# byteowlz/kokorox

Measured on AMD Instinct MI355X. Metric: real-time factor (audio-s/wall-s), 24 kHz, batch=64, higher is better.
Workload: dtype f32 in / out, f32 accumulate; products on split operands: f16f8 (a_hi b_hi on f16 MFMAs, the cross terms a_lo b_hi + a_hi b_lo of the 7 / 11-tap convs on e4m3 scaled MFMAs: ~17 significant bits per product; every other conv f16x3: ~22) -- wider than the bf16 BASELINE configs[2] names, inside the 1e-; 1 GPU; batch=64/GPU synthetic 128-phoneme utterances (T=130), durations pinned 3,3,3,4 -> F=422 frames = 10.55 s each, noise on, inputs in HBM; batch_per_gpu=64, frames=422, parallelism=utterance-sharded x1, one-time weight broadcast

## Files before the change

### kokorox_amd/build.py

```python
from __future__ import annotations

import os
import subprocess
import sys

HERE = os.path.dirname(os.path.abspath(__file__))
CSRC = os.path.join(HERE, "csrc")
LIB_DIR = os.path.join(HERE, "lib")
LIB_PATH = os.path.join(LIB_DIR, "libkokorox_hip.so")
TEST_LIB_PATH = os.path.join(LIB_DIR, "libkokorox_hip_test.so")
TEST_SOURCES = ["test_hooks.hip"]
SOURCES = ["conv_plan.hip", "conv_mfma.hip", "conv_f16x3.hip", "conv_f16x3_da.hip", "conv_f16x3_da_p1.hip", "conv_f16x3_da_w2.hip", "conv_f16x3_da_s16.hip", "conv_f16x3_da_f8.hip", "conv_f16x3_da_pre.hip", "conv_f16x3_pre.hip", "conv_f16x3_dapn.hip", "conv_f16x3_dag.hip", "kernels_misc.hip", "model.hip", "api.hip", "dispatcher.hip", "onnx_import.cpp"]
HEADERS = ["kx_common.h", "kx_error.h", "conv_epilogue.h", "conv_f16x3_common.h"]
_PUB = os.path.join("..", "..", "include", "kokorox_hip.h")
_PUB_TEST = os.path.join("..", "..", "include", "kokorox_hip_test.h")
EXTRA_DEPS = {"model.hip": ["onnx_import.h", "model.h", _PUB], "api.hip": ["model.h", "kx_handle.h", "api_guard.h", _PUB],
              "dispatcher.hip": ["model.h", "kx_handle.h", "dispatcher_core.h", _PUB],
              "test_hooks.hip": ["model.h", "kx_handle.h", "api_guard.h", _PUB, _PUB_TEST], "onnx_import.cpp": ["onnx_import.h"], "conv_f16x3_da_p1.hip": ["conv_f16x3_da.hip"], "conv_f16x3_da_w2.hip": ["conv_f16x3_da.hip"], "conv_f16x3_da_s16.hip": ["conv_f16x3_da.hip"], "conv_f16x3_da_f8.hip": ["conv_f16x3_da.hip"], "conv_f16x3_da_pre.hip": ["conv_f16x3_da.hip"]}
FLAGS = ["-O3", "--offload-arch=gfx950", "-fPIC", "-std=c++17", "-Wall", "-Wno-unused-result"]


def _hipcc() -> str:
    for cand in (os.environ.get("HIPCC"), "/opt/rocm/bin/hipcc", "hipcc"):
        if cand and (os.path.isabs(cand) and os.path.exists(cand) or not os.path.isabs(cand)):
            return cand
    return "hipcc"


def _newer(target: str, deps) -> bool:
    if not os.path.exists(target):
        return False
    t = os.path.getmtime(target)
    return all(os.path.getmtime(d) <= t for d in deps)


LAST_BUILD = {"compiled": [], "reused": [], "linked": False}


def build_library(force: bool = False, verbose: bool = False) -> str:
    LAST_BUILD["compiled"], LAST_BUILD["reused"], LAST_BUILD["linked"] = [], [], False
    os.makedirs(LIB_DIR, exist_ok=True)
# ... 40 lines not shown
```

### kokorox_amd/csrc/conv_f16x3.hip

```cpp
#include "conv_f16x3_common.h"

namespace kx {

template <int BM, int BN, int WM, int WN, int ACT, int TK, bool PF, int VT>
__global__ __launch_bounds__(WM * WN * 64, (WM * WN == 8) ? 4 : ((BM / WM / 32) * (BN / WN / 32) > 6 ? 2 : 3))
void conv1d_f16x3_kernel(const ConvArgs a) {
    constexpr int MT = BM / WM / 32;
    constexpr int NT = BN / WN / 32;
    constexpr int NWV = WM * WN;
    static_assert((NWV == 4 || NWV == 8) && MT >= 1 && NT >= 1, "4 or 8 waves per workgroup");
    static_assert(VT == 1 || (VT <= TK && PF), "virtual taps need TK >= VT and the prefetching build");
    extern __shared__ __attribute__((aligned(16))) unsigned char smem16[];

    const int tid = threadIdx.x;
    const int lane = tid & 63;
    const int wave = __builtin_amdgcn_readfirstlane(tid >> 6);
    const int wm = wave / WN, wn = wave % WN;
    const int r = lane & 31, h = lane >> 5;
    const int b = blockIdx.z, ct = blockIdx.y;
    int tile_x = blockIdx.x;
    if (a.xcd_swizzle && gridDim.x >= 16) {
        const int nx = gridDim.x;
        const int off = (int)(((long)nx * (blockIdx.y + (long)gridDim.y * blockIdx.z)) & 7);
        const int cls = (blockIdx.x + off) & 7;
// ... 364 lines not shown
    else if (bm == 32 && bn == 256 && wm == 1 && wn == 4)
        launch_inst16<32, 256, 1, 4>(p, a, B, s);
    else
        throw Error(1, "conv1d f16x3: no such LDS-DMA form");
}

void launch_conv(const ConvPlan& p, const ConvArgs& a, int B, hipStream_t s) {
    if (p.form == FORM_F32) {
        launch_conv1d(a, p.bm, B, p.cols, s);
        return;
    }
    KX_REQUIRE(a.n_chunks16 == (a.Cin + CK16 - 1) / CK16 && a.w16 != nullptr, "conv1d f16x3: weights not packed");
    KX_REQUIRE(a.epi != EPI_GELU_NEW || p.vt > 1 || p.form == FORM_DAG || p.form == FORM_DAGN,
               "conv1d f16x3: gelu epilogue exists only for k=1 GEMMs with >= 48 input channels");
    KX_REQUIRE(p.merged == (a.merge_T > 0), "conv1d f16x3: merged columns do not match the plan");
    if (p.cols <= 0) return;
    switch (p.form) {
        case FORM_LDS: launch_lds(p, a, B, s); return;
        case FORM_DAG:
        case FORM_DAGN: launch_conv1d_f16x3_dag(p, a, B, s); return;
        case FORM_DAPN: launch_conv1d_f16x3_dapn(a, B, p.cols, s); return;
        case FORM_DA_PRE: launch_conv16_da_pre(p, a, B, s); return;
        case FORM_DA_S16: launch_conv16_da_s16(p, a, B, s); return;
        case FORM_DA_F8: launch_conv16_da_f8(p, a, B, s); return;
        case FORM_DA:
            if (p.p1) {
                launch_conv16_da_p1(p, a, B, s);
                return;
            }
            [[fallthrough]];
        case FORM_DA_W2: {
            static const int dephase = getenv("KX_DEPHASE") ? atoi(getenv("KX_DEPHASE")) : 0;
            static const int dephase_mode = getenv("KX_DEPHASE_MODE") ? atoi(getenv("KX_DEPHASE_MODE")) : 1;
            ConvArgs d;
            const ConvArgs* ap = &a;
            if (dephase > 0 && p.bn == 256) {
                d = a;
                const long grid_n = (long)((p.cols + 255) / 256) * ((a.Cout + 127) / 128) * B;
                const double tile_cycles = (double)a.n_chunks16 * a.K * 8 * 96 * 2.5 + 50000.0;
                d.dephase_cycles = grid_n >= 1024 ? (int)(tile_cycles * dephase / 1000.0) : 0;
                d.dephase_mode = dephase_mode;
                ap = &d;
            }
            if (p.form == FORM_DA_W2)
                launch_conv16_da_w2(p, *ap, B, s);
            else
                launch_conv16_da(p, *ap, B, s);
// ... 172 lines not shown
```

### kokorox_amd/csrc/conv_f16x3_da.hip

```cpp
#include "conv_f16x3_common.h"
#include <type_traits>


#ifndef KX_F8_RAW_AUX
#define KX_F8_RAW_AUX 0
#endif
#ifndef KX_F8_HWCOS
#define KX_F8_HWCOS 1
#endif

namespace kx {

template <int I, int N, class F>
__device__ __forceinline__ void static_for(F&& f) {
    if constexpr (I < N) {
        f(std::integral_constant<int, I>{});
        static_for<I + 1, N>(f);
    }
}

template <int KT, int RH, int RC, int RAW>
struct F8Sched {
    static constexpr int HS = (KT - 1) / 2, NG = (KT + 1) / 4, NC = 2 * NG;
    static constexpr int cross_of(int p) {
        if (p & 1) return -1;
        if (p <= 2 * (NG - 1)) return p / 2;
        if (p >= KT - 1 - 2 * (NG - 1)) return NC - 1 - (KT - 1 - p) / 2;
        return -1;
// ... 11 lines not shown
                n += 2;
                st_h[p + RH <= KT - 1 ? sc * KT + p + RH : (sc + 1) * KT + p % RH] = n;
                const int c = cross_of(p);
                if (c >= 0) {
                    n += 4;
                    st_x[sc * NC + c + RC] = n;
                }
            }
            n += RAW;
        }
        return result < 63 ? result : 63;
    }
    static constexpr int cum(int NB, int first, int n) {
        int t = 0;
        for (int r = 0; r < n; ++r) t += cross_of((first + r) / NB) >= 0 ? 3 : 1;
        return t;
    }
    static constexpr int hu_before(int NB, int NA, int HU, int first, int I0, int rel) {
        return rel > I0 ? ((cum(NB, first, rel) - cum(NB, first, I0)) * HU) / (cum(NB, first, NA) - cum(NB, first, I0)) : 0;
    }
};

template <int ACT, int KT, int NTT, bool P1, bool W2 = false, bool S16 = false, bool PRE = false, bool BF = false, bool F8 = false>
__global__ __launch_bounds__(256, (NTT == 8 || S16) ? 2 : 3) void conv1d_f16x3_da_kernel(const ConvArgs a) {
    static_assert(!BF || P1, "BF: a form of the reduced-precision kernels only");
    static_assert(!F8 || (S16 && KT % 4 == 3), "F8: a form of the S16 loop; tap groups of four with one padding slot");
    constexpr bool HWC = F8 && KX_F8_HWCOS;
    static_assert(!PRE || (!P1 && !S16 && ACT == ACT_NONE), "PRE: the activation lives in the image; f16x3 forms on 32x32x16 only");
    static_assert(!W2 || (KT >= 3 && (KT & 1) && NTT == 8), "W2: odd compile-time tap counts on the 256-column tile");
    static_assert(!S16 || (KT >= 3 && (KT & 1) && !P1 && !W2), "S16: odd compile-time tap counts, three MFMAs per product, 4 x 1 waves");
    static_assert(NTT == 8 || NTT == 4 || (NTT == 6 && S16), "tile widths: 256, 128, and 192 columns in the S16 form");
    constexpr int BM = 128, NT = NTT, BN = 32 * NT;
    constexpr bool W64 = KT > 0;
    constexpr bool SPLIT = W64 && BN % 128 == 0;
    constexpr int NJF = W64 ? (SPLIT ? BN / 128 : (BN + 64) / 128) : (BN + 128) / 128;
    constexpr int NJ = NJF + (SPLIT ? 1 : 0);
    constexpr int HU = 8 * NJF + (SPLIT ? 4 : 0);
    constexpr int XWp = W64 ? BN + 64 : BN + 128;
    static_assert(!W64 || SPLIT || (BN + 64) % 128 == 0, "the window is whole 64-column blocks in pairs, or ends in a split block");
    constexpr int XBUF = 4 * XWp;
    constexpr int tap_units = 4 * BM;
    extern __shared__ __attribute__((aligned(16))) unsigned char smem16[];
    uint4* Xs = reinterpret_cast<uint4*>(smem16);

    const int tid = threadIdx.x;
    const int lane = tid & 63;
    const int wave = __builtin_amdgcn_readfirstlane(tid >> 6);
    const int r = lane & 31, h = lane >> 5;
    auto pack_pair = [](float v0, float v1, unsigned& hi_pk, unsigned& lo_pk) __attribute__((always_inline)) {
        if constexpr (BF) {
            auto rne = [](float x) __attribute__((always_inline)) {
                unsigned u = __builtin_bit_cast(unsigned, x);
                u += 0x7fffu + ((u >> 16) & 1u);
                return u >> 16;
            };
            hi_pk = rne(v0) | (rne(v1) << 16);
            lo_pk = 0u;
        } else if constexpr (F8) {
            split_pair_f8(v0, v1, hi_pk, lo_pk);
        } else {
            split_pair(v0, v1, hi_pk, lo_pk);
        }
// ... 67 lines not shown
    const int K = KT > 0 ? KT : a.K, dil = a.dil;
    const int n_chunks = a.n_chunks16;
    const int n_steps = n_chunks * K;
    const float* xb = a.x + (long)b * a.x_bs;
    const int p0 = t0 - a.pad;
    const bool has_norm = a.nmean != nullptr;
    const int up2 = a.in_up2;
    const int Lsrc = up2 ? ((Lin + 1) >> 1) : Lin;

    f32x16 acc[1][NT];
#pragma unroll
    for (int j = 0; j < NT; ++j)
#pragma unroll
        for (int e = 0; e < 16; ++e) acc[0][j][e] = 0.f;
    constexpr int NB16 = S16 ? 2 * NT : 1;
    f32x4v acc16[2][NB16];
#pragma unroll
    for (int i = 0; i < 2; ++i)
#pragma unroll
        for (int j = 0; j < NB16; ++j) acc16[i][j] = f32x4v{0.f, 0.f, 0.f, 0.f};

    const int g = wave & 1, jb = wave >> 1;
    float raw[NJ][8];
    float praw[4];
    int xoff[NJ];
    unsigned okmask = 0;
    auto blk_col = [&](int j) __attribute__((always_inline)) { return (SPLIT && j == NJF) ? 64 * 2 * NJF : 64 * (jb + 2 * j); };
#pragma unroll
    for (int j = 0; j < NJ; ++j) {
        const int p = p0 + lane + blk_col(j);
        okmask |= (p >= 0 && p < Lin) ? (1u << j) : 0u;
        int pi = up2 ? (p >> 1) : p;
        pi = pi < 0 ? 0 : (pi >= Lsrc ? Lsrc - 1 : pi);
        xoff[j] = pi;
    }
    using u32x4 = __attribute__((ext_vector_type(4))) unsigned;
    constexpr int NLD = PRE ? (4 * XWp) / 256 : 1;
    static_assert(!PRE || (4 * XWp) % 256 == 0, "PRE: whole rounds of 256 lanes");
    u32x4 rawq[NLD];
    unsigned qoff[NLD];
    unsigned okq = 0;
    const buf_rsrc xq = make_buf(PRE ? reinterpret_cast<const char*>(a.x16) + (long)b * a.x16_bs : reinterpret_cast<const char*>(a.x));
    const unsigned chunk_bytes = PRE ? 64u * (unsigned)a.x16_ld : 0u;
    const buf_rsrc xrow = make_buf(xb);
    if constexpr (PRE) {
#pragma unroll
        for (int i = 0; i < NLD; ++i) {
            const int idx = tid + 256 * i, plane = idx / XWp, u = idx - plane * XWp;
            const int p = p0 + u;
            okq |= (p >= 0 && p < Lin) ? (1u << i) : 0u;
            const int pc = p < 0 ? 0 : (p >= Lin ? Lin - 1 : p);
            qoff[i] = 16u * (unsigned)(plane * a.x16_ld + pc);
        }
    }
    const int cmax_in = a.Cin - 1;
    const float* nm_src = has_norm ? a.nmean + (long)b * a.n_bs : xb;
    const float* ns_src = has_norm ? a.nscale + (long)b * a.n_bs : xb;
    const float* nh_src = has_norm ? a.nshift + (long)b * a.n_bs : xb;
    auto load_params = [&](int ch, float (&pv)[4]) __attribute__((always_inline)) {
        const int c = ch * CK16 + g * 8 + (lane & 7);
        const int cc = c < cmax_in ? c : cmax_in;
        const float m = nm_src[cc], sc = ns_src[cc], sh = nh_src[cc];
        const bool cvalid = c <= cmax_in;
        pv[0] = has_norm ? m : 0.f;
        pv[1] = cvalid ? (has_norm ? sc : 1.f) : 0.f;
        pv[2] = (cvalid && has_norm) ? sh : 0.f;
        pv[3] = (ACT == ACT_SNAKE) ? a.alpha[cc] : 1.f;
    };
    auto load_raw = [&](int ch) __attribute__((always_inline)) {
        if constexpr (PRE) {
#pragma unroll
            for (int i = 0; i < NLD; ++i)
                rawq[i] = __builtin_bit_cast(u32x4, __builtin_amdgcn_raw_buffer_load_b128(xq, qoff[i], (unsigned)ch * chunk_bytes, 0));
            return;
        }
        load_params(ch, praw);
        if constexpr (F8) {
#pragma unroll
            for (int c = 0; c < 8; ++c) {
                const int ci = ch * CK16 + g * 8 + c;
                const unsigned so = (unsigned)__builtin_amdgcn_readfirstlane(ci < cmax_in ? ci : cmax_in) * (4u * (unsigned)a.x_ld);
#pragma unroll
                for (int j = 0; j < NJF; ++j) raw[j][c] = __builtin_bit_cast(float, __builtin_amdgcn_raw_buffer_load_b32(xrow, 4u * (unsigned)xoff[j], so, KX_F8_RAW_AUX));
            }
            if constexpr (SPLIT) {
#pragma unroll
                for (int c = 0; c < 4; ++c) {
                    const int ci = ch * CK16 + g * 8 + jb * 4 + c;
                    const unsigned so = (unsigned)__builtin_amdgcn_readfirstlane(ci < cmax_in ? ci : cmax_in) * (4u * (unsigned)a.x_ld);
                    raw[NJF][c] = __builtin_bit_cast(float, __builtin_amdgcn_raw_buffer_load_b32(xrow, 4u * (unsigned)xoff[NJF], so, KX_F8_RAW_AUX));
                }
            }
            return;
        }
#pragma unroll
        for (int c = 0; c < 8; ++c) {
            const int ci = ch * CK16 + g * 8 + c;
            const float* row = xb + (long)(ci < cmax_in ? ci : cmax_in) * a.x_ld;
#pragma unroll
            for (int j = 0; j < NJF; ++j) raw[j][c] = row[xoff[j]];
        }
        if constexpr (SPLIT) {
#pragma unroll
            for (int c = 0; c < 4; ++c) {
                const int ci = ch * CK16 + g * 8 + jb * 4 + c;
                raw[NJF][c] = (xb + (long)(ci < cmax_in ? ci : cmax_in) * a.x_ld)[xoff[NJF]];
            }
        }
    };
    struct Oct { float m[8], s[8], h[8], al[8], ial[8]; };
    auto unpack_params = [&](const float (&pv)[4], Oct& o) __attribute__((always_inline)) {
        const float al_or_rcp = (lane & 8) ? 1.0f / pv[3] : pv[3];
#pragma unroll
// ... 26 lines not shown
        const float al_or_rcp = (lane & 8) ? 1.0f / pv[3] : pv[3];
        const float keep = pok ? a.x_prescale : 0.f;
        unsigned hp[2], lp[2];
#pragma unroll
        for (int c2 = 0; c2 < 2; ++c2) {
            float y2[2];
#pragma unroll
            for (int q = 0; q < 2; ++q) {
                const int c = 2 * c2 + q, cl = jb * 4 + c;
                const float m = __builtin_bit_cast(float, __builtin_amdgcn_readlane(__builtin_bit_cast(int, pv[0]), cl));
                const float sc = __builtin_bit_cast(float, __builtin_amdgcn_readlane(__builtin_bit_cast(int, pv[1]), cl));
                const float sh = __builtin_bit_cast(float, __builtin_amdgcn_readlane(__builtin_bit_cast(int, pv[2]), cl));
                const float al = __builtin_bit_cast(float, __builtin_amdgcn_readlane(__builtin_bit_cast(int, al_or_rcp), cl));
                const float ial = __builtin_bit_cast(float, __builtin_amdgcn_readlane(__builtin_bit_cast(int, al_or_rcp), cl + 8));
                const float y = act_in(__builtin_fmaf(x8[c] - m, sc, sh), a.slope, al, ial);
                y2[q] = y * keep;
            }
            pack_pair(y2[0], y2[1], hp[c2], lp[c2]);
        }
        uint2* Xw2 = reinterpret_cast<uint2*>(Xb);
        Xw2[((0 * 2 + g) * XWp + u) * 2 + jb] = make_uint2(hp[0], hp[1]);
        if constexpr (!P1) Xw2[((1 * 2 + g) * XWp + u) * 2 + jb] = make_uint2(lp[0], lp[1]);
    };
    auto pre_unit = [&](const int i, uint4* Xb) __attribute__((always_inline)) {
        const u32x4 z = {0u, 0u, 0u, 0u};
        const u32x4 v = ((okq >> i) & 1u) ? rawq[i] : z;
        Xb[tid + 256 * i] = __builtin_bit_cast(uint4, v);
    };
    auto stage_from_raw = [&](uint4* Xb, int ch) __attribute__((always_inline)) {
        if constexpr (PRE) {
#pragma unroll
            for (int i = 0; i < NLD; ++i) pre_unit(i, Xb);
            return;
        }
        Oct o;
        unpack_params(praw, o);
#pragma unroll
        for (int j = 0; j < NJF; ++j) emit8(Xb, ch, lane + blk_col(j), raw[j], o, ((okmask >> j) & 1u) != 0u);
        if constexpr (SPLIT) emit4(Xb, ch, lane + blk_col(NJF), raw[NJ - 1], praw, ((okmask >> NJF) & 1u) != 0u);
    };

#ifdef KX_DA_NO_XFORM
    auto keep_elem = [&](const int hh) __attribute__((always_inline)) {
        const int U = hh / 2, half = hh & 1;
        const bool split = SPLIT && U >= 4 * NJF;
        const int j = split ? NJF : U % NJF, cr = split ? 2 * (U - 4 * NJF) + half : 2 * (U / NJF) + half;
        asm volatile("" ::"v"(raw[j][cr]), "v"(praw[0]), "v"(praw[1]), "v"(praw[2]), "v"(praw[3]));
    };
#endif
    float al_rcp_x = 1.f;
    float y_carry = 0.f;
    float xt_ = 0.f, xz_ = 0.f;
    auto xform_a = [&](const int U, const int half, int ch) __attribute__((always_inline)) {
        const bool split = SPLIT && U >= 4 * NJF;
        const int j = split ? NJF : U % NJF, cr = split ? 2 * (U - 4 * NJF) + half : 2 * (U / NJF) + half;
        const int cq = split ? jb * 4 + cr : cr;
        if (U == 0 && half == 0) al_rcp_x = (lane & 8) ? 1.0f / praw[3] : praw[3];
        const float m = __builtin_bit_cast(float, __builtin_amdgcn_readlane(__builtin_bit_cast(int, praw[0]), cq));
        const float sc = __builtin_bit_cast(float, __builtin_amdgcn_readlane(__builtin_bit_cast(int, praw[1]), cq));
        const float sh = __builtin_bit_cast(float, __builtin_amdgcn_readlane(__builtin_bit_cast(int, praw[2]), cq));
        xt_ = __builtin_fmaf(raw[j][cr] - m, sc, sh);
        asm volatile("" : "+v"(xt_));
        if (ACT == ACT_SNAKE && HWC) {
            const float al = __builtin_bit_cast(float, __builtin_amdgcn_readlane(__builtin_bit_cast(int, al_rcp_x), cq));
            xz_ = (al * xt_) * 0.318309886183790672f;
        } else if (ACT == ACT_SNAKE) {
            const float al = __builtin_bit_cast(float, __builtin_amdgcn_readlane(__builtin_bit_cast(int, al_rcp_x), cq));
            const float t = al * xt_;
            const float n = rintf(t * 0.318309886183790672f);
            float rr = fmaf(n, -3.14159274101257324f, t);
            rr = fmaf(n, 8.74227765734758578e-08f, rr);
            xz_ = rr * rr;
        }
    };
    auto xform_b = [&]() __attribute__((always_inline)) {
        if (ACT == ACT_SNAKE && HWC) {
            xz_ = __builtin_fmaf(-0.5f, __builtin_amdgcn_cosf(xz_), 0.5f);
        } else if (ACT == ACT_SNAKE) {
            const float z = xz_;
            float pp = fmaf(z, -3.6197402550897095e-06f, 1.3928599946666651e-04f);
            pp = fmaf(z, pp, -3.1722760759294033e-03f);
            pp = fmaf(z, pp, 4.4443082064390182e-02f);
            pp = fmaf(z, pp, -3.3333304524421692e-01f);
            pp = fmaf(z, pp, 1.0f);
            xz_ = z * pp;
        }
    };
    auto xform_c = [&](const int U, const int half, uint4* Xb, int ch) __attribute__((always_inline)) {
        const bool split = SPLIT && U >= 4 * NJF;
        const int j = split ? NJF : U % NJF;
        const int c2 = split ? jb * 2 + (U - 4 * NJF) : U / NJF;
        const int cq = 2 * c2 + half;
        float y;
        if (ACT == ACT_SNAKE) {
            const float ial = __builtin_bit_cast(float, __builtin_amdgcn_readlane(__builtin_bit_cast(int, al_rcp_x), cq + 8));
            y = fmaf(ial, xz_, xt_);
        } else {
            y = in_act<ACT>(xt_, a.slope, 1.f, 1.f);
        }
        const float keep = ((okmask >> j) & 1u) ? a.x_prescale : 0.f;
        y = y * keep;
        if (half == 0) {
            y_carry = y;
        } else {
            unsigned hp, lp;
            pack_pair(y_carry, y, hp, lp);
            const int u = lane + blk_col(j);
            unsigned* Xw = reinterpret_cast<unsigned*>(Xb);
            Xw[((0 * 2 + g) * XWp + u) * 4 + c2] = hp;
            if constexpr (!P1) Xw[((1 * 2 + g) * XWp + u) * 4 + c2] = lp;
        }
    };

    const uint4* wlane = reinterpret_cast<const uint4*>(a.w16) + (long)ct * n_steps * tap_units + h * BM + wave * 32 + r;
    auto load_A = [&](int s, u32x4& a_hi, u32x4& a_lo) __attribute__((always_inline)) {
        const int sc = s < n_steps ? s : n_steps - 1;
        const uint4* p = wlane + (long)sc * tap_units;
        asm volatile("global_load_dwordx4 %0, %1, off" : "=v"(a_hi) : "v"(p) : "memory");
        if constexpr (!P1) asm volatile("global_load_dwordx4 %0, %1, off" : "=v"(a_lo) : "v"(p + 2 * BM) : "memory");
    };
    constexpr int APL = P1 ? 1 : 2;
    auto wait_vm = [&](int age) __attribute__((always_inline)) {
        if (age >= 60) asm volatile("s_waitcnt vmcnt(60)" ::: "memory");
        else if (age >= 34) asm volatile("s_waitcnt vmcnt(34)" ::: "memory");
        else if (age >= 32) asm volatile("s_waitcnt vmcnt(32)" ::: "memory");
        else if (age >= 30) asm volatile("s_waitcnt vmcnt(30)" ::: "memory");
        else if (age >= 28) asm volatile("s_waitcnt vmcnt(28)" ::: "memory");
        else if (age >= 26) asm volatile("s_waitcnt vmcnt(26)" ::: "memory");
        else if (age >= 24) asm volatile("s_waitcnt vmcnt(24)" ::: "memory");
        else if (age >= 22) asm volatile("s_waitcnt vmcnt(22)" ::: "memory");
// ... 743 lines not shown
                                   ncols, Lout, tile_x * 2, stat_scr, wide_scr);
        conv_store_group<EPI_ROWS>(a, *reinterpret_cast<f32x16(*)[1][4]>(&acc[0][4]), a.w_unscale, b, ct * BM + wave * 32, t0 + 128, r,
                                   h, ncols, Lout, tile_x * 2 + 1, stat_scr, wide_scr);
    } else {
        conv_store_group<EPI_ROWS>(a, acc, a.w_unscale, b, ct * BM + wave * 32, t0, r, h, ncols, Lout, tile_x, stat_scr, wide_scr);
    }
#ifdef KX_DA_STAMPS
    if (a.stamps && tid == 0) {
        const unsigned lin = blockIdx.x + gridDim.x * (blockIdx.y + gridDim.y * blockIdx.z);
        unsigned long long* o = a.stamps + (unsigned long long)lin * 8;
        o[0] = st0; o[1] = st1; o[2] = st2;
        __builtin_amdgcn_s_waitcnt(0);
        o[3] = __builtin_amdgcn_s_memrealtime();
        o[4] = __builtin_amdgcn_s_getreg(63492);
        o[5] = __builtin_readcyclecounter() - cyc0;
        o[6] = F8 ? acc_wait : __builtin_amdgcn_s_getreg(63508);
        o[7] = acc_bar;
    }
#endif
}

template <int ACT, int KT, int NTT, bool P1 = false, bool W2 = false, bool S16 = false, bool PRE = false, bool BF = false, bool F8 = false>
static void launch_da_inst(const ConvArgs& a, int B, int max_cols, hipStream_t s) {
    auto kern = conv1d_f16x3_da_kernel<ACT, KT, NTT, P1, W2, S16, PRE, BF, F8>;
    constexpr int BN = 32 * NTT;
    constexpr size_t lds_x = 16 * (size_t)2 * 4 * (BN + 128), lds_scr = 4 * 32 * 33 * sizeof(float2);
    constexpr size_t lds = lds_x > lds_scr ? lds_x : lds_scr;
    KX_REQUIRE(a.stride == 1 && a.merge_T == 0 && (a.K - 1) * a.dil + 256 <= 384, "conv1d f16x3 da: launch not eligible");
    dim3 grid((max_cols + BN - 1) / BN, (a.Cout + 127) / 128, B);
    KX_REQUIRE(grid.x > 0 && grid.y > 0 && grid.y < 65536 && B > 0 && B < 65536, "conv1d f16x3 da: bad grid");
    if (a.tile_prefix) {
        KX_REQUIRE(a.flat_ny == (int)grid.y && a.flat_B == B && a.flat_bn_host == BN && a.flat_tiles_host > 0 &&
                       (long)a.flat_tiles_host * grid.y < (1L << 30),
                   "conv1d f16x3 da: flat tile list does not match the launch");
        grid = dim3((unsigned)a.flat_tiles_host * grid.y, 1, 1);
    }
    hipLaunchKernelGGL(kern, grid, dim3(256), lds, s, a);
    KX_HIP(hipGetLastError());
}

template <int NTT, bool P1, bool BF>
static void launch_da_4x1(const ConvPlan& p, const ConvArgs& a, int B, hipStream_t s) {
#ifdef KX_DA_AUDIT
    if (p.act == ACT_SNAKE) launch_da_inst<ACT_SNAKE, 11, 8, P1, false, false, false, BF>(a, B, p.cols, s);
    else launch_da_inst<ACT_LEAKY, 0, 4, P1, false, false, false, BF>(a, B, p.cols, s);
    return;
#endif
// ... 29 lines not shown
```

### kokorox_amd/csrc/conv_f16x3_da_f8.hip

```cpp
#define KX_DA_UNIT
#include "conv_f16x3_da.hip"

namespace kx {

void launch_conv16_da_f8(const ConvPlan& p, const ConvArgs& a, int B, hipStream_t s) {
    KX_REQUIRE(p.form == FORM_DA_F8 && a.w8x != nullptr && (p.kt == 11 || p.kt == 7 || p.kt == 3) && a.K == p.kt && (a.K - 1) * a.dil <= 64 &&
                   a.act == ACT_SNAKE && !a.prec1 && a.n_chunks16 >= 2 && (a.n_chunks16 & 1) == 0,
               "conv1d f16x3 da f8: launch not eligible");
    KX_REQUIRE(p.bn == 192 || p.bn == 128, "conv1d f16x3 da f8: tile of 192 or 128 columns");
    KX_REQUIRE((long)a.Cin * a.x_ld * 4 < (1L << 32), "conv1d f16x3 da f8: input tensor of one utterance beyond 4 GiB");
    if (p.kt == 11) {
        if (p.bn == 192) launch_da_inst<ACT_SNAKE, 11, 6, false, false, true, false, false, true>(a, B, p.cols, s);
        else launch_da_inst<ACT_SNAKE, 11, 4, false, false, true, false, false, true>(a, B, p.cols, s);
    } else if (p.kt == 7) {
        if (p.bn == 192) launch_da_inst<ACT_SNAKE, 7, 6, false, false, true, false, false, true>(a, B, p.cols, s);
        else launch_da_inst<ACT_SNAKE, 7, 4, false, false, true, false, false, true>(a, B, p.cols, s);
    } else {
        if (p.bn == 192) launch_da_inst<ACT_SNAKE, 3, 6, false, false, true, false, false, true>(a, B, p.cols, s);
        else launch_da_inst<ACT_SNAKE, 3, 4, false, false, true, false, false, true>(a, B, p.cols, s);
    }
}

}
```

### kokorox_amd/csrc/conv_plan.hip

```cpp
#include "kx_common.h"

namespace kx {

static bool da_eligible(int BM, int K, int dil, int stride, bool merged) {
    return BM == 128 && stride == 1 && !merged && (K - 1) * dil + 256 <= 384;
}

static bool f8_taps(int K, int dil) { return (K == 11 || K == 7 || K == 3) && (K - 1) * dil <= 64; }

static bool s16_shape(int BM, int K, int dil, int stride, int act, int n_chunks16, bool merged, int pmode) {
    const bool taps = K == 11 || (K == 7 && dil == 1) || (pmode == 2 && f8_taps(K, dil));
    return BM == 128 && stride == 1 && !merged && pmode != 1 && act == ACT_SNAKE && taps && (K - 1) * dil <= 64 && n_chunks16 >= 2 &&
           (n_chunks16 & 1) == 0;
}

bool conv16_f8_layer(int BM, int rows, int K, int n_chunks16) {
    return BM == 128 && f8_taps(K, 1) && (K != 3 || rows <= 256) && n_chunks16 >= 2 && (n_chunks16 & 1) == 0;
}

ConvPlan conv_plan(const ConvLaunch& c) {
    ConvPlan p{};
    p.bm = c.BM;
    p.act = c.act;
    p.vt = 1;
// ... 35 lines not shown
        const long tiles = (long)((p.cols + 127) / 128) * ((c.rows + 127) / 128);
        if (route != FORCE_LDS && !c.norm && c.store != ST_UPSCATTER) {
            const long wgs = tiles * (p.merged ? 1 : c.B);
            const bool narrow_ok = (c.x_bs * c.B + 16L * c.x_ld) * 4 < (1L << 31);
            p.form = narrow_ok && 2 * wgs <= c.cus ? FORM_DAGN : FORM_DAG;
            p.bn = p.form == FORM_DAGN ? 32 : 128;
            return p;
        }
        p.form = FORM_LDS;
        p.bn = 128;
        p.wm = 2;
        p.wn = 2;
        p.pf = 1;
        p.vt = tiles > 2L * c.cus ? 2 : 3;
        return p;
    }

    const bool da = route != FORCE_LDS && da_eligible(c.BM, c.K, c.dil, c.stride, p.merged);
    const bool small = (long)((p.cols + 255) / 256) * ((c.rows + 127) / 128) * c.B < 256;
    if (route != FORCE_LDS && !(c.force & FORCE_NO_S16) && s16_shape(c.BM, c.K, c.dil, c.stride, c.act, c.n_chunks16, p.merged, pmode)) {
        p.form = pmode == 2 ? FORM_DA_F8 : FORM_DA_S16;
        p.kt = c.K;
        p.bn = small && route != FORCE_DA ? 128 : 192;
        set_stats(64);
    } else if (!da || (route != FORCE_DA && c.cols <= 160 && !stats)) {
        p.form = FORM_LDS;
        const bool short_seq = c.cols <= 160 && !stats;
        p.bn = !short_seq && !small ? 256 : 128;
        p.wm = !short_seq && small ? 4 : 2;
        p.wn = !short_seq && small ? 1 : 2;
        p.pf = c.stride == 1 && (c.K - 1) * c.dil <= 128;
        set_stats(p.bn / p.wn);
    } else {
        p.bn = small && route != FORCE_DA ? 128 : 256;
        set_stats(128);
        const bool w64 = (c.K - 1) * c.dil <= 64;
        if (p.pre) {
            const bool narrow = p.bn == 128 && !c.prec1 && c.rows % 32 == 0 && c.K <= 12 && c.epi == EPI_NONE &&
                                (c.store == ST_NORMAL || c.store == ST_UPSCATTER) && (long)c.n_chunks16 * c.K < 5000;
            p.form = narrow ? FORM_DAPN : FORM_DA_PRE;
            p.act = ACT_NONE;
            p.kt = c.K == 3 && w64 ? 3 : 0;
        } else {
            const bool unrolled = w64 && ((c.act == ACT_SNAKE && (c.K == 11 || c.K == 7 || c.K == 3)) || (c.act == ACT_LEAKY && c.K == 3));
            p.kt = unrolled ? c.K : 0;
            p.p1 = c.prec1 != 0;
// ... 11 lines not shown
```

### kokorox_amd/csrc/kx_common.h

```cpp
#pragma once
#include <hip/hip_runtime.h>

#include <cmath>
#include <cstdint>
#include <cstring>
#include <cstdio>
#include <stdexcept>
#include <string>

#include <atomic>
#include <mutex>

#include "kx_error.h"

namespace kx {

constexpr int KX_MAX_DEVICES = 64;

struct DynLdsLimit {
    std::atomic<size_t> limit[KX_MAX_DEVICES];
    std::mutex mu;
    DynLdsLimit() {
        for (auto& l : limit) l.store(64 * 1024);
    }
// ... 84 lines not shown
    int dbg;
    const int* tile_prefix;
    int flat_ny;
    int flat_B;
    int flat_tiles_host, flat_bn_host;
    const void* x16;
    long x16_bs;
    int x16_ld;
};

enum ConvMode { CONV_F32 = 0, CONV_F16X3 = 1, CONV_F16X3_LDS = 2, CONV_F16X3_DA = 3, CONV_F16 = 4, CONV_BF16 = 5, CONV_F16F8 = 6 };
enum ConvForm {
    FORM_F32 = 0,
    FORM_LDS,
    FORM_DAG,
    FORM_DAGN,
    FORM_DA,
    FORM_DA_W2,
    FORM_DA_S16,
    FORM_DA_F8,
    FORM_DA_PRE,
    FORM_DAPN,
};
enum ConvForce { FORCE_LDS = 1, FORCE_DA = 2, FORCE_DA_4X1 = 4, FORCE_NO_S16 = 8 };

struct ConvLaunch {
    int mode;
    int prec1;
    int f8;
    int BM, rows, n_chunks16, K, dil, stride, pad, act, in_up2, store, accum, epi;
    int norm;
    int stats;
    int image;
    int merge_T;
    long x_bs;
    int x_ld;
    int B, cols;
    int cus;
    int force;
};
struct ConvPlan {
    int form;
    int bm, act, kt, wm, wn, vt, pf, p1, bf;
    int bn;
    int cols;
    int merged;
    int pre;
    int stat_cols, stat_tiles;
    int flat_bn;
};
ConvPlan conv_plan(const ConvLaunch& c);
bool conv16_f8_layer(int BM, int rows, int K, int n_chunks16);
void launch_conv(const ConvPlan& p, const ConvArgs& a, int B, hipStream_t s);
int conv16_cu_count();
int cu_count_override();

size_t conv16_pre_image_bytes(int Cin, int x_ld);
void launch_split_image(const ConvArgs& a, int B, int Lmax, void* img, long img_bs, hipStream_t s);

void launch_tile_prefix(LenMap len, int extra, int bn, int B, int* out, hipStream_t s);

inline int conv_pick_bm(int rows) { return rows >= 128 ? 128 : (rows > 32 ? 64 : 32); }

void launch_conv1d(const ConvArgs& a, int BM, int B, int max_cols, hipStream_t s);

struct PackSrc {
    const float* p[3];
    int rows[3];
};
void launch_pack_conv(const PackSrc& src, float* dst, int Cout, int Cin, int K, int BM, hipStream_t s);
void launch_pack_convT(const float* w, float* dst, int Cin, int Cout, int s, int BM, hipStream_t s_);
size_t packed_conv_floats(int rows, int Cin, int K, int BM);

void launch_conv16_da(const ConvPlan& p, const ConvArgs& a, int B, hipStream_t s);
void launch_conv16_da_p1(const ConvPlan& p, const ConvArgs& a, int B, hipStream_t s);
void launch_conv16_da_w2(const ConvPlan& p, const ConvArgs& a, int B, hipStream_t s);
void launch_conv16_da_s16(const ConvPlan& p, const ConvArgs& a, int B, hipStream_t s);
void launch_conv16_da_f8(const ConvPlan& p, const ConvArgs& a, int B, hipStream_t s);
void launch_conv16_da_pre(const ConvPlan& p, const ConvArgs& a, int B, hipStream_t s);
void launch_conv1d_f16x3_dapn(const ConvArgs& a, int B, int max_cols, hipStream_t s);
void launch_conv1d_f16x3_dag(const ConvPlan& p, const ConvArgs& a, int B, hipStream_t s);
size_t packed_conv16_halves(int rows, int Cin, int K, int BM);
float device_absmax(const float* p, long n, hipStream_t s);
int pick_weight_shift(float absmax);
void launch_pack_conv16(const PackSrc& src, void* dst, int Cout, int Cin, int K, int BM, float wscale, hipStream_t s);
void launch_pack_convT16(const float* w, void* dst, int Cin, int Cout, int sd, int BM, float wscale, hipStream_t s);
void launch_image_to_bf16(const void* w16, void* dst, size_t n_halves, hipStream_t s);
size_t packed_conv8x_bytes(int rows, int Cin, int K);
void launch_pack_conv8x(const void* w16, void* dst, int rows, int Cin, int K, hipStream_t s);

void launch_vec_add(const float* a, const float* b, float* out, int n, hipStream_t s);
void launch_transpose_whh(const float* whh, float* out, hipStream_t s);

void launch_albert_embed(const int64_t* ids, long ids_stride, const float* word, const float* type0,
                         const float* pos, float* out, long bs, int ld, const int* lens, int B, int Tmax,
                         int n_vocab, unsigned* bad_id, hipStream_t s);
void launch_embed(const int64_t* ids, long ids_stride, const float* table, int C, float* out, long bs, int ld,
                  const int* lens, int B, int Tmax, int n_vocab, unsigned* bad_id, hipStream_t s);

enum LnMode { LN_PLAIN = 0, LN_AFFINE = 1, LN_ADA = 2 };
void launch_layernorm_ch(const float* x, float* y, long bs, int ld, int C, LenMap len, int B, int Lmax,
// ... 67 lines not shown
```

### kokorox_amd/hip_koko.py

```python
from __future__ import annotations

import ctypes as C
import os
from typing import List, Optional, Sequence

import numpy as np

_HERE = os.path.dirname(os.path.abspath(__file__))
LIB_PATH = os.path.join(_HERE, "lib", "libkokorox_hip.so")

PACK_F32_MONO, PACK_F32_STEREO, PACK_PCM16_MONO = 0, 1, 2
KX_OK, KX_ERR_INVALID, KX_ERR_IO, KX_ERR_DEVICE, KX_ERR_STATE = 0, 1, 2, 3, 4
KX_FLAG_NOISE_OFF = 1
KX_FLAG_TAPS = 2
STYLE_DIM = 256
SAMPLES_PER_FRAME = 600

_lib = None


class KokoroxHipError(RuntimeError):
    def __init__(self, code: int, msg: str):
        super().__init__(f"kokorox_hip error {code}: {msg}")
        self.code = code
# ... 528 lines not shown
           device=0, mode=None, pre=False):
    lib = load_test_library()
    if mode is None:
        mode = CONV_F32 if os.environ.get("KOKOROX_CONV", "") == "f32" else CONV_F16X3
    x, w = _f32(x), _f32(w)
    B, Cin, L = x.shape
    k = w.shape[2]
    if transposed:
        Cout = w.shape[1]
        Lout = (L - 1) * stride - 2 * pad + k
    else:
        Cout = w.shape[0]
        Lout = (L + 2 * pad - dil * (k - 1) - 1) // stride + 1
    y = np.zeros((B, Cout, Lout), dtype=np.float32)
    bias, alpha, norm = _f32(bias), _f32(alpha), _f32(norm)
    _err_call(lib.kx_test_conv1d, device, _ptr(x), B, Cin, L, _ptr(w), _ptr(bias), Cout, k, stride, pad, dil,
              1 if transposed else 0, act, float(slope), _ptr(alpha), _ptr(norm), _ptr(y), Lout, mode | (0x100 if pre else 0))
    return y


CONV_LAUNCH_FIELDS = ("mode", "prec1", "f8", "BM", "rows", "n_chunks16", "K", "dil", "stride", "pad", "act", "in_up2", "store", "accum",
                      "epi", "norm", "stats", "image", "merge_T", "x_bs", "x_ld", "B", "cols", "cus", "force")
CONV_PLAN_FIELDS = ("form", "bm", "act", "kt", "wm", "wn", "vt", "pf", "p1", "bf", "bn", "cols", "merged", "pre", "stat_cols",
                    "stat_tiles", "flat_bn")
CONV_FORMS = ("F32", "LDS", "DAG", "DAGN", "DA", "DA_W2", "DA_S16", "DA_F8", "DA_PRE", "DAPN")


def conv_plan(**launch):
    lib = load_test_library()
    unknown = set(launch) - set(CONV_LAUNCH_FIELDS)
    assert not unknown, unknown
    src = np.array([int(launch.get(f, 0)) for f in CONV_LAUNCH_FIELDS], dtype=np.int64)
    out = np.zeros(len(CONV_PLAN_FIELDS), dtype=np.int64)
    _err_call(lib.kx_test_conv_plan, _ptr(src), len(src), _ptr(out), len(out))
    plan = dict(zip(CONV_PLAN_FIELDS, (int(v) for v in out)))
    plan["form"] = CONV_FORMS[plan["form"]]
    return plan


def conv_transpose(x, w, bias=None, stride=6, act=1, slope=0.1, resid=None, up_off=0, mode=1, pre=False, device=0):
    lib = load_test_library()
    x, w = _f32(x), _f32(w)
    B, Cin, L = x.shape
    Cout, k = w.shape[1], w.shape[2]
    assert k == 2 * stride
    pad = (k - stride) // 2
    Lout = (L - 1) * stride - 2 * pad + k
# ... 67 lines not shown
```

Measured before the change: 6619 x realtime.

## Add narrow 32-column halo window variant of the F8 snake conv kernel

```diff
diff --git a/kokorox_amd/build.py b/kokorox_amd/build.py
--- a/kokorox_amd/build.py
+++ b/kokorox_amd/build.py
@@ -10,13 +10,13 @@
 LIB_PATH = os.path.join(LIB_DIR, "libkokorox_hip.so")
 TEST_LIB_PATH = os.path.join(LIB_DIR, "libkokorox_hip_test.so")
 TEST_SOURCES = ["test_hooks.hip"]
-SOURCES = ["conv_plan.hip", "conv_mfma.hip", "conv_f16x3.hip", "conv_f16x3_da.hip", "conv_f16x3_da_p1.hip", "conv_f16x3_da_w2.hip", "conv_f16x3_da_s16.hip", "conv_f16x3_da_f8.hip", "conv_f16x3_da_pre.hip", "conv_f16x3_pre.hip", "conv_f16x3_dapn.hip", "conv_f16x3_dag.hip", "kernels_misc.hip", "model.hip", "api.hip", "dispatcher.hip", "onnx_import.cpp"]
+SOURCES = ["conv_plan.hip", "conv_mfma.hip", "conv_f16x3.hip", "conv_f16x3_da.hip", "conv_f16x3_da_p1.hip", "conv_f16x3_da_w2.hip", "conv_f16x3_da_s16.hip", "conv_f16x3_da_f8.hip", "conv_f16x3_da_f8n.hip", "conv_f16x3_da_pre.hip", "conv_f16x3_pre.hip", "conv_f16x3_dapn.hip", "conv_f16x3_dag.hip", "kernels_misc.hip", "model.hip", "api.hip", "dispatcher.hip", "onnx_import.cpp"]
 HEADERS = ["kx_common.h", "kx_error.h", "conv_epilogue.h", "conv_f16x3_common.h"]
 _PUB = os.path.join("..", "..", "include", "kokorox_hip.h")
 _PUB_TEST = os.path.join("..", "..", "include", "kokorox_hip_test.h")
 EXTRA_DEPS = {"model.hip": ["onnx_import.h", "model.h", _PUB], "api.hip": ["model.h", "kx_handle.h", "api_guard.h", _PUB],
               "dispatcher.hip": ["model.h", "kx_handle.h", "dispatcher_core.h", _PUB],
-              "test_hooks.hip": ["model.h", "kx_handle.h", "api_guard.h", _PUB, _PUB_TEST], "onnx_import.cpp": ["onnx_import.h"], "conv_f16x3_da_p1.hip": ["conv_f16x3_da.hip"], "conv_f16x3_da_w2.hip": ["conv_f16x3_da.hip"], "conv_f16x3_da_s16.hip": ["conv_f16x3_da.hip"], "conv_f16x3_da_f8.hip": ["conv_f16x3_da.hip"], "conv_f16x3_da_pre.hip": ["conv_f16x3_da.hip"]}
+              "test_hooks.hip": ["model.h", "kx_handle.h", "api_guard.h", _PUB, _PUB_TEST], "onnx_import.cpp": ["onnx_import.h"], "conv_f16x3_da_p1.hip": ["conv_f16x3_da.hip"], "conv_f16x3_da_w2.hip": ["conv_f16x3_da.hip"], "conv_f16x3_da_s16.hip": ["conv_f16x3_da.hip"], "conv_f16x3_da_f8.hip": ["conv_f16x3_da.hip"], "conv_f16x3_da_f8n.hip": ["conv_f16x3_da.hip"],"conv_f16x3_da_pre.hip": ["conv_f16x3_da.hip"]}
 FLAGS = ["-O3", "--offload-arch=gfx950", "-fPIC", "-std=c++17", "-Wall", "-Wno-unused-result"]
 
 
diff --git a/kokorox_amd/csrc/conv_f16x3.hip b/kokorox_amd/csrc/conv_f16x3.hip
--- a/kokorox_amd/csrc/conv_f16x3.hip
+++ b/kokorox_amd/csrc/conv_f16x3.hip
@@ -410,7 +410,10 @@
         case FORM_DAPN: launch_conv1d_f16x3_dapn(a, B, p.cols, s); return;
         case FORM_DA_PRE: launch_conv16_da_pre(p, a, B, s); return;
         case FORM_DA_S16: launch_conv16_da_s16(p, a, B, s); return;
-        case FORM_DA_F8: launch_conv16_da_f8(p, a, B, s); return;
+        case FORM_DA_F8:
+            if (p.win == 32) launch_conv16_da_f8n(p, a, B, s);
+            else launch_conv16_da_f8(p, a, B, s);
+            return;
         case FORM_DA:
             if (p.p1) {
                 launch_conv16_da_p1(p, a, B, s);
diff --git a/kokorox_amd/csrc/conv_f16x3_da.hip b/kokorox_amd/csrc/conv_f16x3_da.hip
--- a/kokorox_amd/csrc/conv_f16x3_da.hip
+++ b/kokorox_amd/csrc/conv_f16x3_da.hip
@@ -4,6 +4,12 @@
 
 #ifndef KX_F8_RAW_AUX
 #define KX_F8_RAW_AUX 0
+#endif
+#ifndef KX_DA_WIN32
+#define KX_DA_WIN32 0
+#endif
+#ifndef KX_DA_KERNEL
+#define KX_DA_KERNEL conv1d_f16x3_da_kernel
 #endif
 #ifndef KX_F8_HWCOS
 #define KX_F8_HWCOS 1
@@ -61,7 +67,7 @@
 };
 
 template <int ACT, int KT, int NTT, bool P1, bool W2 = false, bool S16 = false, bool PRE = false, bool BF = false, bool F8 = false>
-__global__ __launch_bounds__(256, (NTT == 8 || S16) ? 2 : 3) void conv1d_f16x3_da_kernel(const ConvArgs a) {
+__global__ __launch_bounds__(256, (NTT == 8 || S16) ? 2 : 3) void KX_DA_KERNEL(const ConvArgs a) {
     static_assert(!BF || P1, "BF: a form of the reduced-precision kernels only");
     static_assert(!F8 || (S16 && KT % 4 == 3), "F8: a form of the S16 loop; tap groups of four with one padding slot");
     constexpr bool HWC = F8 && KX_F8_HWCOS;
@@ -71,12 +77,24 @@
     static_assert(NTT == 8 || NTT == 4 || (NTT == 6 && S16), "tile widths: 256, 128, and 192 columns in the S16 form");
     constexpr int BM = 128, NT = NTT, BN = 32 * NT;
     constexpr bool W64 = KT > 0;
-    constexpr bool SPLIT = W64 && BN % 128 == 0;
-    constexpr int NJF = W64 ? (SPLIT ? BN / 128 : (BN + 64) / 128) : (BN + 128) / 128;
+    constexpr bool W32 = KX_DA_WIN32 != 0;
+    static_assert(!W32 || (F8 && W64 && (NT == 6 || NT == 4)), "narrow window: the F8 forms only");
+    constexpr bool SPLIT = W64 && (W32 ? NT == 6 : BN % 128 == 0);
+    constexpr int NJF = W64 ? (W32 ? 1 : (SPLIT ? BN / 128 : (BN + 64) / 128)) : (BN + 128) / 128;
     constexpr int NJ = NJF + (SPLIT ? 1 : 0);
-    constexpr int HU = 8 * NJF + (SPLIT ? 4 : 0);
+    constexpr int HU = 8 * NJF + (SPLIT ? 4 : 0) + (W32 ? 2 : 0);
+    constexpr int UT = 4 * NJF + (SPLIT ? 2 : 0);
+    static_assert(!W32 || 64 * 2 * NJF + (SPLIT ? 64 : 0) == BN, "narrow window: the tail starts at column BN");
+    constexpr bool ROT = W32 && SPLIT && KT != 7;
+    struct Unit { bool tail, split; int j, e2; };
+    auto unit_of = [](const int U) __attribute__((always_inline)) {
+        const bool tail = W32 && U == UT;
+        if (ROT) return Unit{tail, U < 4 && (U & 1), (U < 4 && (U & 1)) ? NJF : 0, tail ? 0 : (U < 4 ? U >> 1 : U - 2)};
+        const bool split = SPLIT && U >= 4 * NJF && !tail;
+        return Unit{tail, split, split ? NJF : U % NJF, tail ? 0 : (split ? U - 4 * NJF : U / NJF)};
+    };
     constexpr int XWp = W64 ? BN + 64 : BN + 128;
-    static_assert(!W64 || SPLIT || (BN + 64) % 128 == 0, "the window is whole 64-column blocks in pairs, or ends in a split block");
+    static_assert(!W64 || SPLIT || W32 || (BN + 64) % 128 == 0,"the window is whole 64-column blocks in pairs, or ends in a split block");
     constexpr int XBUF = 4 * XWp;
     constexpr int tap_units = 4 * BM;
     extern __shared__ __attribute__((aligned(16))) unsigned char smem16[];
@@ -190,6 +208,7 @@
 
     const int g = wave & 1, jb = wave >> 1;
     float raw[NJ][8];
+    float rawt[2] = {0.f, 0.f};
     float praw[4];
     int xoff[NJ];
     unsigned okmask = 0;
@@ -202,6 +221,17 @@
         pi = pi < 0 ? 0 : (pi >= Lsrc ? Lsrc - 1 : pi);
         xoff[j] = pi;
     }
+    int xoff_t = 0;
+    const int tail_cq = jb * 4 + 2 * (lane >> 5);
+    if constexpr (W32) {
+        const int p = p0 + BN + (lane & 31);
+        okmask |= (p >= 0 && p < Lin) ? (1u << NJ) : 0u;
+        int pi = up2 ? (p >> 1) : p;
+        xoff_t = pi < 0 ? 0 : (pi >= Lsrc ? Lsrc - 1 : pi);
+    }
+    auto tail_par = [&](float v, const int q, const int up) __attribute__((always_inline)) {
+        return __builtin_bit_cast(float, __builtin_amdgcn_ds_bpermute(4 * (tail_cq + q + up), __builtin_bit_cast(int, v)));
+    };
     using u32x4 = __attribute__((ext_vector_type(4))) unsigned;
     constexpr int NLD = PRE ? (4 * XWp) / 256 : 1;
     static_assert(!PRE || (4 * XWp) % 256 == 0, "PRE: whole rounds of 256 lanes");
@@ -246,7 +276,7 @@
         if constexpr (F8) {
 #pragma unroll
             for (int c = 0; c < 8; ++c) {
-                const int ci = ch * CK16 + g * 8 + c;
+                const int ci = ch * CK16 + g * 8 + (ROT ? (c < 4 ? jb * 4 + c : c - jb * 4) : c);
                 const unsigned so = (unsigned)__builtin_amdgcn_readfirstlane(ci < cmax_in ? ci : cmax_in) * (4u * (unsigned)a.x_ld);
 #pragma unroll
                 for (int j = 0; j < NJF; ++j) raw[j][c] = __builtin_bit_cast(float, __builtin_amdgcn_raw_buffer_load_b32(xrow, 4u * (unsigned)xoff[j], so, KX_F8_RAW_AUX));
@@ -257,6 +287,14 @@
                     const int ci = ch * CK16 + g * 8 + jb * 4 + c;
                     const unsigned so = (unsigned)__builtin_amdgcn_readfirstlane(ci < cmax_in ? ci : cmax_in) * (4u * (unsigned)a.x_ld);
                     raw[NJF][c] = __builtin_bit_cast(float, __builtin_amdgcn_raw_buffer_load_b32(xrow, 4u * (unsigned)xoff[NJF], so, KX_F8_RAW_AUX));
+                }
+            }
+            if constexpr (W32) {
+#pragma unroll
+                for (int q = 0; q < 2; ++q) {
+                    const int ci = ch * CK16 + g * 8 + tail_cq + q;
+                    const unsigned ro = (unsigned)(ci < cmax_in ? ci : cmax_in) * (4u * (unsigned)a.x_ld);
+                    rawt[q] = __builtin_bit_cast(float, __builtin_amdgcn_raw_buffer_load_b32(xrow, 4u * (unsigned)xoff_t + ro, 0u, KX_F8_RAW_AUX));
                 }
             }
             return;
@@ -329,6 +367,23 @@
         Xw2[((0 * 2 + g) * XWp + u) * 2 + jb] = make_uint2(hp[0], hp[1]);
         if constexpr (!P1) Xw2[((1 * 2 + g) * XWp + u) * 2 + jb] = make_uint2(lp[0], lp[1]);
     };
+    auto emit_tail = [&](uint4* Xb, const float (&pv)[4]) __attribute__((always_inline)) {
+        const float al_or_rcp = (lane & 8) ? 1.0f / pv[3] : pv[3];
+        const float keep = ((okmask >> NJ) & 1u) ? a.x_prescale : 0.f;
+        float y2[2];
+#pragma unroll
+        for (int q = 0; q < 2; ++q) {
+            const float y = act_in(__builtin_fmaf(rawt[q] - tail_par(pv[0], q, 0), tail_par(pv[1], q, 0), tail_par(pv[2], q, 0)), a.slope,
+                                   tail_par(al_or_rcp, q, 0), tail_par(al_or_rcp, q, 8));
+            y2[q] = y * keep;
+        }
+        unsigned hp, lp;
+        pack_pair(y2[0], y2[1], hp, lp);
+        const int u = BN + (lane & 31), c2 = tail_cq >> 1;
+        unsigned* Xw = reinterpret_cast<unsigned*>(Xb);
+        Xw[((0 * 2 + g) * XWp + u) * 4 + c2] = hp;
+        if constexpr (!P1) Xw[((1 * 2 + g) * XWp + u) * 4 + c2] = lp;
+    };
     auto pre_unit = [&](const int i, uint4* Xb) __attribute__((always_inline)) {
         const u32x4 z = {0u, 0u, 0u, 0u};
         const u32x4 v = ((okq >> i) & 1u) ? rawq[i] : z;
@@ -343,26 +398,45 @@
         Oct o;
         unpack_params(praw, o);
 #pragma unroll
-        for (int j = 0; j < NJF; ++j) emit8(Xb, ch, lane + blk_col(j), raw[j], o, ((okmask >> j) & 1u) != 0u);
+        for (int j = 0; j < NJF; ++j) {
+            if constexpr (ROT) {
+                float x8[8];
+#pragma unroll
+                for (int c = 0; c < 8; ++c) x8[c] = jb ? raw[j][c ^ 4] : raw[j][c];
+                emit8(Xb, ch, lane + blk_col(j), x8, o, ((okmask >> j) & 1u) != 0u);
+            } else {
+                emit8(Xb, ch, lane + blk_col(j), raw[j], o, ((okmask >> j) & 1u) != 0u);
+            }
+        }
         if constexpr (SPLIT) emit4(Xb, ch, lane + blk_col(NJF), raw[NJ - 1], praw, ((okmask >> NJF) & 1u) != 0u);
+        if constexpr (W32) emit_tail(Xb, praw);
     };
 
 #ifdef KX_DA_NO_XFORM
     auto keep_elem = [&](const int hh) __attribute__((always_inline)) {
         const int U = hh / 2, half = hh & 1;
-        const bool split = SPLIT && U >= 4 * NJF;
-        const int j = split ? NJF : U % NJF, cr = split ? 2 * (U - 4 * NJF) + half : 2 * (U / NJF) + half;
-        asm volatile("" ::"v"(raw[j][cr]), "v"(praw[0]), "v"(praw[1]), "v"(praw[2]), "v"(praw[3]));
+        const Unit un = unit_of(U);
+        const bool tail = un.tail;
+        const int j = un.j, cr = 2 * un.e2 + half;
+        asm volatile("" ::"v"(tail ? rawt[half] : raw[j][cr]), "v"(praw[0]), "v"(praw[1]), "v"(praw[2]), "v"(praw[3]));
     };
 #endif
     float al_rcp_x = 1.f;
     float y_carry = 0.f;
     float xt_ = 0.f, xz_ = 0.f;
     auto xform_a = [&](const int U, const int half, int ch) __attribute__((always_inline)) {
-        const bool split = SPLIT && U >= 4 * NJF;
-        const int j = split ? NJF : U % NJF, cr = split ? 2 * (U - 4 * NJF) + half : 2 * (U / NJF) + half;
-        const int cq = split ? jb * 4 + cr : cr;
+        const Unit un = unit_of(U);
+        const bool tail = un.tail, split = un.split;
+        const int j = un.j, cr = 2 * un.e2 + half;
+        const int cq = (split || (ROT && cr < 4)) ? jb * 4 + cr : (ROT ? cr - jb * 4 : cr);
         if (U == 0 && half == 0) al_rcp_x = (lane & 8) ? 1.0f / praw[3] : praw[3];
+        static_assert(!W32 || (ACT == ACT_SNAKE && HWC), "narrow window: the hardware-cosine snake of the F8 forms");
+        if (tail) {
+            xt_ = __builtin_fmaf(rawt[half] - tail_par(praw[0], half, 0), tail_par(praw[1], half, 0), tail_par(praw[2], half, 0));
+            asm volatile("" : "+v"(xt_));
+            xz_ = (tail_par(al_rcp_x, half, 0) * xt_) * 0.318309886183790672f;
+            return;
+        }
         const float m = __builtin_bit_cast(float, __builtin_amdgcn_readlane(__builtin_bit_cast(int, praw[0]), cq));
         const float sc = __builtin_bit_cast(float, __builtin_amdgcn_readlane(__builtin_bit_cast(int, praw[1]), cq));
         const float sh = __builtin_bit_cast(float, __builtin_amdgcn_readlane(__builtin_bit_cast(int, praw[2]), cq));
@@ -394,12 +468,15 @@
         }
     };
     auto xform_c = [&](const int U, const int half, uint4* Xb, int ch) __attribute__((always_inline)) {
-        const bool split = SPLIT && U >= 4 * NJF;
-        const int j = split ? NJF : U % NJF;
-        const int c2 = split ? jb * 2 + (U - 4 * NJF) : U / NJF;
-        const int cq = 2 * c2 + half;
+        const Unit un = unit_of(U);
+        const bool tail = un.tail, split = un.split;
+        const int j = tail ? NJ : un.j;
+        const int c2 = tail ? (tail_cq >> 1) : ((split || (ROT && un.e2 < 2)) ? jb * 2 + un.e2 : (ROT ? un.e2 - jb * 2 : un.e2));
+        const int cq = tail ? 0 : 2 * c2 + half;
         float y;
-        if (ACT == ACT_SNAKE) {
+        if (ACT == ACT_SNAKE && tail) {
+            y = fmaf(tail_par(al_rcp_x, half, 8), xz_, xt_);
+        } else if (ACT == ACT_SNAKE) {
             const float ial = __builtin_bit_cast(float, __builtin_amdgcn_readlane(__builtin_bit_cast(int, al_rcp_x), cq + 8));
             y = fmaf(ial, xz_, xt_);
         } else {
@@ -412,7 +489,7 @@
         } else {
             unsigned hp, lp;
             pack_pair(y_carry, y, hp, lp);
-            const int u = lane + blk_col(j);
+            const int u = tail ? BN + (lane & 31) : lane + blk_col(j);
             unsigned* Xw = reinterpret_cast<unsigned*>(Xb);
             Xw[((0 * 2 + g) * XWp + u) * 4 + c2] = hp;
             if constexpr (!P1) Xw[((1 * 2 + g) * XWp + u) * 4 + c2] = lp;
@@ -1202,7 +1279,7 @@
 
 template <int ACT, int KT, int NTT, bool P1 = false, bool W2 = false, bool S16 = false, bool PRE = false, bool BF = false, bool F8 = false>
 static void launch_da_inst(const ConvArgs& a, int B, int max_cols, hipStream_t s) {
-    auto kern = conv1d_f16x3_da_kernel<ACT, KT, NTT, P1, W2, S16, PRE, BF, F8>;
+    auto kern = KX_DA_KERNEL<ACT, KT, NTT, P1, W2, S16, PRE, BF, F8>;
     constexpr int BN = 32 * NTT;
     constexpr size_t lds_x = 16 * (size_t)2 * 4 * (BN + 128), lds_scr = 4 * 32 * 33 * sizeof(float2);
     constexpr size_t lds = lds_x > lds_scr ? lds_x : lds_scr;
diff --git a/kokorox_amd/csrc/conv_f16x3_da_f8.hip b/kokorox_amd/csrc/conv_f16x3_da_f8.hip
--- a/kokorox_amd/csrc/conv_f16x3_da_f8.hip
+++ b/kokorox_amd/csrc/conv_f16x3_da_f8.hip
@@ -4,7 +4,7 @@
 namespace kx {
 
 void launch_conv16_da_f8(const ConvPlan& p, const ConvArgs& a, int B, hipStream_t s) {
-    KX_REQUIRE(p.form == FORM_DA_F8 && a.w8x != nullptr && (p.kt == 11 || p.kt == 7 || p.kt == 3) && a.K == p.kt && (a.K - 1) * a.dil <= 64 &&
+    KX_REQUIRE(p.form == FORM_DA_F8 && p.win == 64 && a.w8x != nullptr && (p.kt == 11 || p.kt == 7 || p.kt == 3) && a.K == p.kt && (a.K - 1) * a.dil <= 64 &&
                    a.act == ACT_SNAKE && !a.prec1 && a.n_chunks16 >= 2 && (a.n_chunks16 & 1) == 0,
                "conv1d f16x3 da f8: launch not eligible");
     KX_REQUIRE(p.bn == 192 || p.bn == 128, "conv1d f16x3 da f8: tile of 192 or 128 columns");
diff --git a/kokorox_amd/csrc/conv_f16x3_da_f8n.hip b/kokorox_amd/csrc/conv_f16x3_da_f8n.hip
--- /dev/null
+++ b/kokorox_amd/csrc/conv_f16x3_da_f8n.hip
@@ -0,0 +1,26 @@
+#define KX_DA_UNIT
+#define KX_DA_WIN32 1
+#define KX_DA_KERNEL conv1d_f16x3_dan_kernel
+#include "conv_f16x3_da.hip"
+
+namespace kx {
+
+void launch_conv16_da_f8n(const ConvPlan& p, const ConvArgs& a, int B, hipStream_t s) {
+    KX_REQUIRE(p.form == FORM_DA_F8 && p.win == 32 && a.w8x != nullptr && (p.kt == 11 || p.kt == 7 || p.kt == 3) && a.K == p.kt &&
+                   (a.K - 1) * a.dil <= 32 && a.act == ACT_SNAKE && !a.prec1 && a.n_chunks16 >= 2 && (a.n_chunks16 & 1) == 0,
+               "conv1d f16x3 da f8n: launch not eligible");
+    KX_REQUIRE(p.bn == 192 || p.bn == 128, "conv1d f16x3 da f8n: tile of 192 or 128 columns");
+    KX_REQUIRE((long)a.Cin * a.x_ld * 4 < (1L << 32), "conv1d f16x3 da f8n: input tensor of one utterance beyond 4 GiB");
+    if (p.kt == 11) {
+        if (p.bn == 192) launch_da_inst<ACT_SNAKE, 11, 6, false, false, true, false, false, true>(a, B, p.cols, s);
+        else launch_da_inst<ACT_SNAKE, 11, 4, false, false, true, false, false, true>(a, B, p.cols, s);
+    } else if (p.kt == 7) {
+        if (p.bn == 192) launch_da_inst<ACT_SNAKE, 7, 6, false, false, true, false, false, true>(a, B, p.cols, s);
+        else launch_da_inst<ACT_SNAKE, 7, 4, false, false, true, false, false, true>(a, B, p.cols, s);
+    } else {
+        if (p.bn == 192) launch_da_inst<ACT_SNAKE, 3, 6, false, false, true, false, false, true>(a, B, p.cols, s);
+        else launch_da_inst<ACT_SNAKE, 3, 4, false, false, true, false, false, true>(a, B, p.cols, s);
+    }
+}
+
+}
diff --git a/kokorox_amd/csrc/conv_plan.hip b/kokorox_amd/csrc/conv_plan.hip
--- a/kokorox_amd/csrc/conv_plan.hip
+++ b/kokorox_amd/csrc/conv_plan.hip
@@ -81,6 +81,7 @@
         p.form = pmode == 2 ? FORM_DA_F8 : FORM_DA_S16;
         p.kt = c.K;
         p.bn = small && route != FORCE_DA ? 128 : 192;
+        if (p.form == FORM_DA_F8) p.win = (c.K - 1) * c.dil <= 32 && !(c.force & FORCE_WIN64) ? 32 : 64;
         set_stats(64);
     } else if (!da || (route != FORCE_DA && c.cols <= 160 && !stats)) {
         p.form = FORM_LDS;
diff --git a/kokorox_amd/csrc/kx_common.h b/kokorox_amd/csrc/kx_common.h
--- a/kokorox_amd/csrc/kx_common.h
+++ b/kokorox_amd/csrc/kx_common.h
@@ -130,7 +130,7 @@
     FORM_DA_PRE,
     FORM_DAPN,
 };
-enum ConvForce { FORCE_LDS = 1, FORCE_DA = 2, FORCE_DA_4X1 = 4, FORCE_NO_S16 = 8 };
+enum ConvForce { FORCE_LDS = 1, FORCE_DA = 2, FORCE_DA_4X1 = 4, FORCE_NO_S16 = 8, FORCE_WIN64 = 16 };
 
 struct ConvLaunch {
     int mode;
@@ -156,6 +156,7 @@
     int pre;
     int stat_cols, stat_tiles;
     int flat_bn;
+    int win;
 };
 ConvPlan conv_plan(const ConvLaunch& c);
 bool conv16_f8_layer(int BM, int rows, int K, int n_chunks16);
@@ -185,6 +186,7 @@
 void launch_conv16_da_w2(const ConvPlan& p, const ConvArgs& a, int B, hipStream_t s);
 void launch_conv16_da_s16(const ConvPlan& p, const ConvArgs& a, int B, hipStream_t s);
 void launch_conv16_da_f8(const ConvPlan& p, const ConvArgs& a, int B, hipStream_t s);
+void launch_conv16_da_f8n(const ConvPlan& p, const ConvArgs& a, int B, hipStream_t s);
 void launch_conv16_da_pre(const ConvPlan& p, const ConvArgs& a, int B, hipStream_t s);
 void launch_conv1d_f16x3_dapn(const ConvArgs& a, int B, int max_cols, hipStream_t s);
 void launch_conv1d_f16x3_dag(const ConvPlan& p, const ConvArgs& a, int B, hipStream_t s);
diff --git a/kokorox_amd/hip_koko.py b/kokorox_amd/hip_koko.py
--- a/kokorox_amd/hip_koko.py
+++ b/kokorox_amd/hip_koko.py
@@ -574,7 +574,7 @@
 CONV_LAUNCH_FIELDS = ("mode", "prec1", "f8", "BM", "rows", "n_chunks16", "K", "dil", "stride", "pad", "act", "in_up2", "store", "accum",
                       "epi", "norm", "stats", "image", "merge_T", "x_bs", "x_ld", "B", "cols", "cus", "force")
 CONV_PLAN_FIELDS = ("form", "bm", "act", "kt", "wm", "wn", "vt", "pf", "p1", "bf", "bn", "cols", "merged", "pre", "stat_cols",
-                    "stat_tiles", "flat_bn")
+                    "stat_tiles", "flat_bn", "win")
 CONV_FORMS = ("F32", "LDS", "DAG", "DAGN", "DA", "DA_W2", "DA_S16", "DA_F8", "DA_PRE", "DAPN")
 
 
```

Measured after the change: 6536 x realtime. 0.988x the previous value.
